# ai3DVision/CP_PFDR_graph_d1

Measured on AMD Instinct MI355X. Metric: PFDR iter/s and Medge-updates/s, 10M-vertex 6-NN graph, 1/2/4/8 MI355X, higher is better.
Workload: dtype f32; 1 GPU; PFDR_graph_quadratic_d1_l1<float>, identity A, l1 + TV, jittered 250x200x200 grid, 6-NN (V=10000000, E=60000000); global_graph=250x200x200, V_per_gpu=10000000, E_per_gpu=60000000, parallelism=single, device_inputs=True, device_bytes=3010452620, relabelled=False, split_incidence_blocks=0, tiled_blocks=39063, record_blocks=39063, slot_patterns=0, sequential_evolution=False, speculation=none, finite=True

## Files before the change

### cp_pfdr_graph_d1_amd/csrc/pfdr_quadratic.hip

```cpp
#include <cstring>
#include <map>
#include <stdexcept>


#include "pfdr_halo.hpp"
#include "pfdr_order.hpp"
#include "pfdr_quadratic_kernels.hpp"
#include "pfdr_sort.hpp"
#include "pfdr_sparse.hpp"

namespace pfdr {

template <typename real>
static void copy_in(DevBuf<real> &d, const void *src, size_t n, int mem, hipStream_t s,
                    HostPins &pins) {
    if (!src || !n) { d.release(); return; }
    d.alloc(n);
    if (mem == PFDR_MEM_DEVICE)
        PFDR_HIP(hipMemcpyAsync(d.p, src, n * sizeof(real), hipMemcpyDeviceToDevice, s));
    else
        pins.copy(d.p, src, n * sizeof(real), hipMemcpyHostToDevice);
}

template <typename real>
// ... 103 lines not shown
    long E_;
    real rho_, condMin_, difTol_, difRcd2_, cap_;
    int prox_, positivity_;
    real lo_, hi_;
    bool Ldiag_;
    bool rec_obj_, rec_dif_, track_;
    static constexpr int xcd_e_ = 64, xcd_v_ = 16;
    bool us_ = true;
    DevBuf<char> mono_ws_;
    bool la_uniform_ = false;
    real la0_ = real(0);
    bool l1_uniform_ = false;
    real l1u_ = real(0);
    const real *la_it() const { return la_uniform_ ? nullptr : La_d1_.p; }
    int evo_ = PFDR_EVOLUTION_AUTO;
    bool seqdif_ = false;
    long tstride_ = 0;
    DevBuf<real> terms_;
    DevBuf<char> dws_;
    ChainSum<real> chain_;
    TermRoute<real> route_;
    std::unique_ptr<Transport> evtr_;
    Transport &etr() { return evtr_ ? *evtr_ : *halo_->tr; }
    void seq_evolution(real *terms, const real *part, hipStream_t s);
    void sweeps(const Ctrl<real> *c);
    static constexpr int kSpecMax = 4;
    bool spec_ = false;
    int sd_ = 2;
    int it0_ = 0;
    DevBuf<R2<real>> xpx_[kSpecMax - 1];
    R2<real> *xpb(int t) { return spec_ && t % sd_ ? xpx_[t % sd_ - 1].p : xp_.p; }
    R2<real> *xr_ = nullptr, *xw_ = nullptr;
    hipStream_t evs_ = nullptr;
    hipStream_t evs() const { return evs_ ? evs_ : stream; }
    hipEvent_t evv_[kSpecMax] = {}, evd_[kSpecMax] = {};
    Ctrl<real> *snap_[2] = {};
    hipEvent_t snapev_[2] = {};
    void body_spec(int i, int n);
    static constexpr long kSeqDifMin = 1L << 17;
    std::unique_ptr<Halo> halo_;
    bool reordered_ = false;
    DevBuf<int> order_, where_, emap_;
    DevBuf<unsigned> eorig_;
    DevBuf<real> amp_orig_;
    DevBuf<int> Eu_, Ev_;
    DevBuf<real> La_d1_, La_l1_, Y_, A_, L_;
    DevBuf<R2<real>> xp_;
    DevBuf<real> diag_, Ga_, invAux_, Th_l1_, absval_, grad_, pre_, xout_;
    DevBuf<real> Z2_, wz_;
    DevBuf<real> A1_;
    DevBuf<R2<real>> gi_;
    DevBuf<real> rr_;
    int vpair_cap_ = 0;
    bool rat_on_ = false;
    real cw_ = real(0);
    DevBuf<real> R_, vpart_, opart_, Obj_, Dif_, red_, csum_;
    DevBuf<double> Rpart_;
    DevBuf<real> Rsum_, xfull_;
    DevBuf<int> lab_;
    DevBuf<real> ampg_;
    long v0_ = 0, Vglob_ = 0;
    DevBuf<long long> ccnt_;
    DevBuf<int> cnt_part_;
    DevBuf<Ctrl<real>> ctrl_;
    Incidence inc_;
    HostPins pins_;
    DevBuf<int> uptr_, blkok_;
    DevBuf<unsigned> mask_, oidx_;
    void build_split();
    bool tiled_ = false;
    DevBuf<Slots12> slots_;
    DevBuf<unsigned char> deg8_;
    DevBuf<unsigned short> luv_;
    DevBuf<int> erec_;
    DevBuf<int> ustart_, tptr_, tstart_, tlen_, tok_, trec_;
    DevBuf<Slots12> ptab_;
    DevBuf<int> prec_;
    void build_tiles();
    void build_patterns(const unsigned short *d2, long n);
    void build_tile_runs();
    Ctrl<real> *hctrl_ = nullptr;
    int nbv_, nbe_, nbn_, rows_nb_, rows_cpb_;
    int it_ = 0;
    bool stopped_ = false;
    int chunk_ = 32;
    int next_print_ = 0;
    bool graphs_ok_ = false;
    bool capturable_ = false;
    std::map<int, hipGraphExec_t> graphs_;
    void run_bodies(int n);
    hipGraphExec_t chunk_graph(int n);
  public:
    void prepare(int iters) override;
  private:
    void drop_graphs() {
        for (auto &kv : graphs_) (void)hipGraphExecDestroy(kv.second);
        graphs_.clear();
    }

    void setup_graph(const pfdr_problem *p);
    void amplitude(bool init);
    void precondition(bool init);
    void gemv_rows(int gate);
    void forward_dense(int gate);
    void gradient();
    void objective();
// ... 610 lines not shown
    k_tile_ustart<<<grid_for(Eint_ + 1), kBlock, 0, s>>>(Eint_, nb, Eu_.p, ustart_.p);
    DevBuf<int> cnt(nb), fill(nb);
    PFDR_HIP(hipMemsetAsync(cnt.p, 0, sizeof(int) * nb, s));
    PFDR_HIP(hipMemsetAsync(fill.p, 0, sizeof(int) * nb, s));
    struct Src { long n; const int *a; const unsigned long long *keys; long rs; };
    const Src src[3] = {{E_, Ev_.p, nullptr, 0},
                        {E_ - Eint_, Eu_.p + Eint_, nullptr, Eint_ - E_},
                        {R, nullptr, halo_ ? halo_->recv_keys.p : nullptr, E_}};
    for (const Src &q : src)
        if (q.n > 0) k_tile_runs_count<<<grid_for(q.n), kBlock, 0, s>>>(q.n, q.a, q.keys, V_, cnt.p);
    PFDR_HIP(hipGetLastError());
    std::vector<int> h(nb), tp((size_t)nb + 1, 0);
    PFDR_HIP(hipMemcpyAsync(h.data(), cnt.p, sizeof(int) * nb, hipMemcpyDeviceToHost, s));
    PFDR_HIP(hipStreamSynchronize(s));
    for (int b = 0; b < nb; b++) tp[b + 1] = tp[b] + h[b];
    const int nruns = tp[nb];
    tptr_.alloc((size_t)nb + 1);
    PFDR_HIP(hipMemcpyAsync(tptr_.p, tp.data(), sizeof(int) * (nb + 1), hipMemcpyHostToDevice, s));
    tstart_.alloc(nruns ? nruns : 1);
    tlen_.alloc(nruns ? nruns : 1);
    for (const Src &q : src)
        if (q.n > 0)
            k_tile_runs_fill<<<grid_for(q.n), kBlock, 0, s>>>(q.n, q.a, q.keys, V_, q.rs, tptr_.p,
                                                              fill.p, tstart_.p, tlen_.p);
    tok_.alloc(nb);
    k_tile_ok<<<grid_for(nb), kBlock, 0, s>>>(V_, nb, inc_.ptr.p, tptr_.p, kTileCap, tok_.p);
    trec_.alloc((size_t)nb * kTileRec);
    k_tile_rec<<<grid_for(nb), kBlock, 0, s>>>(nb, ustart_.p, tptr_.p, tstart_.p, tlen_.p, tok_.p,
                                               trec_.p);
    deg8_.alloc(V_);
    k_tile_deg<<<grid_for(V_), kBlock, 0, s>>>(V_, inc_.ptr.p, deg8_.p);
    PFDR_HIP(hipGetLastError());
    PFDR_HIP(hipMemcpyAsync(h.data(), tok_.p, sizeof(int) * nb, hipMemcpyDeviceToHost, s));
    PFDR_HIP(hipStreamSynchronize(s));
    long n = 0, nr = 0;
    for (int x : h) {
        n += x != 0;
        nr += x == 2;
    }
    tiled_blocks = n;
    record_blocks = nr;
    const char *e = getenv("PFDR_VPAIR");
    if (sizeof(real) == 4 && nr == nb && !(e && e[0] == '0')) {
        DevBuf<int> ent(nb);
        k_rec_entries<<<grid_for(nb), kBlock, 0, s>>>(V_, nb, inc_.ptr.p, tok_.p, ent.p);
        PFDR_HIP(hipGetLastError());
        PFDR_HIP(hipMemcpyAsync(h.data(), ent.p, sizeof(int) * nb, hipMemcpyDeviceToHost, s));
        PFDR_HIP(hipStreamSynchronize(s));
        const int cap = std::max(1, *std::max_element(h.begin(), h.end()));
        const size_t per_wg = 2 * (size_t)cap * sizeof(real) + 2048;
        if (per_wg * 7 <= 160 * 1024) vpair_cap_ = cap;
        vertex_pair = vpair_cap_;
    }
}

template <typename real>
void QuadSession<real>::build_patterns(const unsigned short *d2, long n) {
    const char *e = getenv("PFDR_TILE_PATTERNS");
    if ((e && e[0] == '0') || !record_blocks) return;
    hipStream_t s = stream;
    const int nb = grid_for(V_);
    const long nr = (long)nb * kPrec;
    std::vector<unsigned long long> hh(nr);
    std::vector<int> rec((size_t)nb * kTileRec);
    {
        DevBuf<unsigned long long> h(nr);
        k_run_hash<<<grid_for(nr), kBlock, 0, s>>>(nb, E_, tok_.p, trec_.p, d2, h.p);
        PFDR_HIP(hipGetLastError());
        PFDR_HIP(hipMemcpyAsync(hh.data(), h.p, sizeof(unsigned long long) * nr,
                                hipMemcpyDeviceToHost, s));
        PFDR_HIP(hipMemcpyAsync(rec.data(), trec_.p, sizeof(int) * rec.size(),
                                hipMemcpyDeviceToHost, s));
        PFDR_HIP(hipStreamSynchronize(s));
    }
    constexpr size_t kMaxPatterns = 65536;
    std::unordered_map<unsigned long long, int> pat;
    std::vector<long long> pA;
    std::vector<int> pLen, pOff, prec(nr, 0);
    std::vector<long long> repA(nr, -1);
    long groups = 0;
    for (long id = 0; id < nr; id++) {
        if (hh[id] == ~0ull) continue;
        auto it = pat.find(hh[id]);
        int pi;
        if (it == pat.end()) {
            const int b = (int)(id / kPrec), q = (int)(id % kPrec);
            const int *r = &rec[(size_t)b * kTileRec];
            const long long A = q == 0 ? r[0] : E_ + r[1 + 2 * q];
            const int len = q == 0 ? r[1] : r[2 + 2 * q];
            pi = (int)pA.size();
            pat.emplace(hh[id], pi);
            pA.push_back(A);
            pLen.push_back(len);
            pOff.push_back((int)groups);
            groups += ((A & 7) + len + 7) / 8;
            if (pat.size() > kMaxPatterns || groups * kSlotGroup > n / 4) return;
        } else {
            pi = it->second;
        }
        prec[id] = pOff[pi];
        repA[id] = pA[pi];
    }
    if (!groups) return;
    {
        DevBuf<long long> dr(nr);
        DevBuf<int> bad(1);
// ... 442 lines not shown
    a.late = fuse_ ? 1 : 0;
    a.E = E_;
    if (tiled_) {
        a.slots = slots_.p; a.trec = trec_.p; a.ptab = ptab_.p; a.prec = prec_.p; a.deg8 = deg8_.p; a.ustart = ustart_.p; a.tptr = tptr_.p; a.tstart = tstart_.p;
        a.tlen = tlen_.p; a.tok = tok_.p;
        a.zs = Z2_.p; a.invAux = invAux_.p; a.a0 = cw_ * la0_;
        a.gi = gi_.p;
    }
    a.l1uni = l1_uniform_ ? 1 : 0;
    a.l1u = l1u_;
    a.terms = seqdif_ ? terms_.p : nullptr;
    a.tmap = seqdif_ && reordered_ ? order_.p : nullptr;
    a.tstride = tstride_;
    a.bbeg = bbeg; a.nb = bend - bbeg; a.xcd = xcd_fit(a.nb, xcd_v_);
    a.bsplit = a.nb; a.bjump = 0;
    return a;
}

template <typename real>
void QuadSession<real>::vertex_sweep(int bbeg, int bend, const Ctrl<real> *c, const char *name,
                                     int bbeg2, int bend2) {
    if (bend <= bbeg) { bbeg = bbeg2; bend = bend2; bbeg2 = bend2 = 0; }
    if (bend <= bbeg) return;
    hipStream_t s = stream;
    VArgs<real> a = vargs(bbeg, bend, c);
    if (bend2 > bbeg2) {
        a.bsplit = bend - bbeg;
        a.bjump = bbeg2 - bend;
        a.nb += bend2 - bbeg2;
        a.xcd = xcd_fit(a.nb, xcd_v_);
    }
    ProfScope ps(prof, name, s);
    if (pad_ && bend2 <= bbeg2) {
        k_vertex_sweep_pad<real><<<xcd_grid(a.nb, a.xcd), kBlock, 0, s>>>(
            a, wzp_.p, pad_nmax_, ends_ ? pidx_.p : nullptr, ends_ ? xpe_.p : nullptr);
        return;
    }
    if (vpair_cap_ && bend2 <= bbeg2 && a.nb >= 2) {
        const int np = a.nb / 2;
        const size_t lb = 2 * (size_t)vpair_cap_ * sizeof(real);
        if (a.nb & 1) {
            VArgs<real> a1 = a;
            a1.bbeg = a.bbeg + a.nb - 1;
            a1.nb = 1;
            a1.bsplit = 1;
            a1.xcd = 0;
            if (zdirect()) k_vertex_sweep<real, 8, true><<<1, kBlock, 0, s>>>(a1);
            else k_vertex_sweep<real, 8><<<1, kBlock, 0, s>>>(a1);
        }
        a.xcd = xcd_fit(np, xcd_v_);
        const int g = xcd_grid(np, a.xcd);
        if (zdirect()) k_vertex_sweep_pair<real, true><<<g, kBlock, lb, s>>>(a, vpair_cap_);
        else k_vertex_sweep_pair<real><<<g, kBlock, lb, s>>>(a, vpair_cap_);
        return;
    }
    if (zdirect())
        k_vertex_sweep<real, 8, true><<<xcd_grid(a.nb, a.xcd), kBlock, 0, s>>>(a);
    else
        k_vertex_sweep<real, 8><<<xcd_grid(a.nb, a.xcd), kBlock, 0, s>>>(a);
}

template <typename real>
void QuadSession<real>::sweeps(const Ctrl<real> *c) {
    hipStream_t s = stream;
    if (overlap_) {
        PFDR_HIP(hipEventRecord(ev_[0], s));
        PFDR_HIP(hipStreamWaitEvent(comm_, ev_[0], 0));
        {
            ProfScope ps(prof, "halo_pull", comm_);
            halo_->pull(xr_, sizeof(R2<real>), comm_);
        }
        PFDR_HIP(hipEventRecord(ev_[1], comm_));
        edge_sweep(elo_, ehi_, c, "edge_sweep");
        PFDR_HIP(hipStreamWaitEvent(s, ev_[1], 0));
        edge_sweep(0, elo_, c, "edge_sweep_b", ehi_, E_);
        PFDR_HIP(hipEventRecord(ev_[2], s));
        PFDR_HIP(hipStreamWaitEvent(comm_, ev_[2], 0));
        {
            ProfScope ps(prof, "halo_push", comm_);
            real *src = zdirect() ? Z2_.p : wz_.p;
            halo_->push(src, src + 2 * E_, sizeof(real), comm_);
        }
        PFDR_HIP(hipEventRecord(ev_[3], comm_));
        vertex_sweep(blo_, bhi_, c, "vertex_sweep");
        PFDR_HIP(hipStreamWaitEvent(s, ev_[3], 0));
        vertex_sweep(0, blo_, c, "vertex_sweep_b", bhi_, nbv_);
    } else {
        if (halo_) {
            ProfScope ps(prof, "halo_pull", s);
            halo_->pull(xr_, sizeof(R2<real>), s);
        }
        edge_sweep(0, E_, c, "edge_sweep");
        if (halo_) {
            ProfScope ps(prof, "halo_push", s);
            real *src = zdirect() ? Z2_.p : wz_.p;
            halo_->push(src, src + 2 * E_, sizeof(real), s);
        }
        vertex_sweep(0, nbv_, c, "vertex_sweep");
    }
}

template <typename real>
void QuadSession<real>::body_spec(int i, int n) {
    hipStream_t s = stream;
    const int t = it0_ + 1 + i;
    const Ctrl<real> *c = ctrl_.p;
// ... 498 lines not shown
```

### cp_pfdr_graph_d1_amd/csrc/pfdr_quadratic_kernels.hpp

```cpp
#pragma once
#include <algorithm>
#include <cmath>
#include <cstring>
#include <memory>
#include <type_traits>

#include "pfdr_graph.hpp"
#include "pfdr_monosum.hpp"
#include "pfdr_session.hpp"

namespace pfdr {

enum AMode : int { A_IDENT = 0, A_DIAG = 1, A_DIRECT = 2, A_ATA = 3 };
enum Prox : int { PROX_NONE = 0, PROX_L1 = 1, PROX_POS = 2, PROX_BOX = 3,
                  PROX_LO = 4, PROX_HI = 5 };
enum Gate : int { GATE_NONE = 0, GATE_ACTIVE = 1, GATE_OBJ = 2,
                  GATE_ACTIVE_OR_OBJ = 3 };

template <typename real> using R2 = typename Vec<real>::v2;

template <typename T, int N>
__device__ __forceinline__ Pk<T, N> ldv(const T *p) {
    return *reinterpret_cast<const Pk<T, N> *>(p);
}
// ... 213 lines not shown
    const int ngv = nt ? rp[nt - 1] : 0;
    int lo = 0, end = nt ? rp[0] : 0, beg = 0;
    for (int b = 0; b < ngv; b += kBlock * GG) {
        Slots12 d[GG];
        Pk<real, VE> x[GG][ZV];
        long base[GG], A[GG];
        int L[GG];
#pragma unroll
        for (int u = 0; u < GG; u++) {
            const int k = min(b + u * kBlock + tid, ngv - 1);
            while (end <= k) {
                beg = end;
                end = rp[++lo];
            }
            A[u] = E + rs[lo];
            L[u] = rl[lo];
            base[u] = (A[u] / G + (k - beg)) * G;
        }
#pragma unroll
        for (int u = 0; u < GG; u++) {
            d[u] = slots[base[u] / G];
#pragma unroll
            for (int z = 0; z < ZV; z++) x[u][z] = ldv<real, VE>(wz + base[u] + z * VE);
        }
#pragma unroll
        for (int u = 0; u < GG; u++)
            if (b + u * kBlock + tid < ngv) {
#pragma unroll
                for (int q = 0; q < G; q++)
                    if (base[u] + q >= A[u] && base[u] + q < A[u] + L[u])
                        lds[slot12(d[u], q)] = x[u][q / VE].v[q % VE];
            }
    }
    __syncthreads();
    int my0 = dinc - dg;
    for (int q = 0; q < w; q++) my0 += wt[q];
    const int my1 = my0 + dg;
    real s = real(0);
    int j = my0;
    for (; j + 4 <= my1; j += 4) {
        const real a0 = lds[j], a1 = lds[j + 1], a2 = lds[j + 2], a3 = lds[j + 3];
        s += ZD ? wv * a0 : a0;
        s += ZD ? wv * a1 : a1;
        s += ZD ? wv * a2 : a2;
        s += ZD ? wv * a3 : a3;
    }
    for (; j < my1; j++) s += ZD ? wv * lds[j] : lds[j];
    return s;
}

constexpr int kRecRuns = 14, kTileRec = 32;
constexpr int kPrec = 16;

template <typename real, bool ZD = false>
__device__ __forceinline__ real tile_sum_rec(int V, long E, int blk, int v,
                                             const unsigned char *__restrict__ deg8,
                                             const Slots12 *__restrict__ slots,
                                             const int *__restrict__ trec,
                                             const real *__restrict__ wz, real *lds, int *wt,
                                             real wv = real(1),
                                             const Slots12 *__restrict__ ptab = nullptr,
                                             const int *__restrict__ prec = nullptr,
                                             bool pre = false, int pre_rv = 0, int pre_pr = 0,
                                             int pre_dg = 0) {
    constexpr int VE = Vec<real>::kPer16B, G = kSlotGroup, ZV = G / VE;
    const int tid = threadIdx.x, lane = tid & (kWave - 1), w = tid / kWave;
    const int dg = pre ? pre_dg : v < V ? deg8[v] : 0;
    const int rv = pre ? pre_rv : lane < kTileRec ? trec[(long)blk * kTileRec + lane] : 0;
    const int pr = pre ? pre_pr : prec && lane < kPrec ? prec[(long)blk * kPrec + lane] : 0;
    int dinc = dg;
#pragma unroll
    for (int o = 1; o < kWave; o <<= 1) {
        const int y = __shfl_up(dinc, o, kWave);
        if (lane >= o) dinc += y;
    }
    if (lane == kWave - 1) wt[w] = dinc;
    const int us = __builtin_amdgcn_readlane(rv, 0), nu = __builtin_amdgcn_readlane(rv, 1);
    const int nt = __builtin_amdgcn_readlane(rv, 2);
    const int st = __shfl(rv, min(3 + 2 * lane, kWave - 1), kWave);
    const int ln = __shfl(rv, min(4 + 2 * lane, kWave - 1), kWave);
    int P = 0;
    if (lane < nt && ln > 0) {
        const long A = E + st;
        P = (int)((A + ln - 1) / G - A / G + 1);
    }
#pragma unroll
    for (int o = 1; o < kWave; o <<= 1) {
        const int y = __shfl_up(P, o, kWave);
        if (lane >= o) P += y;
    }
    const int ngv = __builtin_amdgcn_readlane(P, kWave - 1);
    const long fu = us / G;
    const int ngu = nu > 0 ? (int)((us + nu - 1) / G - fu + 1) : 0;
    const int tot = ngu + ngv;
    for (int b = 0; b < tot; b += 2 * kBlock) {
        Slots12 d[2];
        Pk<real, VE> x[2][ZV];
        long gb[2], lo[2], hi[2];
        int pg[2];
#pragma unroll
        for (int u = 0; u < 2; u++) {
            const int k = min(b + u * kBlock + tid, tot - 1);
            const int kv = k - ngu;
            int r = 0;
            for (int q = 0; q < nt; q++) r += __builtin_amdgcn_readlane(P, q) <= kv;
            r = min(r, kWave - 1);
            const int sr = __shfl(st, r, kWave), lr = __shfl(ln, r, kWave);
            const int pb = __shfl(P, max(r - 1, 0), kWave);
            const int pv = __shfl(pr, min(r + 1, kWave - 1), kWave);
            if (k < ngu) {
                gb[u] = fu + k;
                lo[u] = us;
                hi[u] = (long)us + nu;
                pg[u] = __builtin_amdgcn_readlane(pr, 0) + k;
            } else {
                const long A = E + sr;
                const int gi = kv - (r > 0 ? pb : 0);
                gb[u] = A / G + gi;
                lo[u] = A;
                hi[u] = A + lr;
                pg[u] = pv + gi;
            }
        }
#pragma unroll
        for (int u = 0; u < 2; u++) {
            d[u] = prec ? ptab[pg[u]] : slots[gb[u]];
#pragma unroll
            for (int z = 0; z < ZV; z++) x[u][z] = ldv<real, VE>(wz + gb[u] * G + z * VE);
        }
#pragma unroll
        for (int u = 0; u < 2; u++)
            if (b + u * kBlock + tid < tot) {
#pragma unroll
                for (int q = 0; q < G; q++) {
                    const long p = gb[u] * G + q;
                    if (p >= lo[u] && p < hi[u]) lds[slot12(d[u], q)] = x[u][q / VE].v[q % VE];
                }
            }
    }
    __syncthreads();
    int my0 = dinc - dg;
    for (int q = 0; q < w; q++) my0 += wt[q];
    const int my1 = my0 + dg;
    real s = real(0);
    int j = my0;
    for (; j + 4 <= my1; j += 4) {
        const real a0 = lds[j], a1 = lds[j + 1], a2 = lds[j + 2], a3 = lds[j + 3];
        s += ZD ? wv * a0 : a0;
        s += ZD ? wv * a1 : a1;
        s += ZD ? wv * a2 : a2;
        s += ZD ? wv * a3 : a3;
    }
    for (; j < my1; j++) s += ZD ? wv * lds[j] : lds[j];
    return s;
}

template <typename real, bool ZD = false>
__device__ __forceinline__ void tile_sum_rec2(int V, long E, int b0, int v0, int v1,
                                              const unsigned char *__restrict__ deg8,
                                              const Slots12 *__restrict__ slots,
                                              const int *__restrict__ trec,
                                              const real *__restrict__ wz, real *lds, int cap,
                                              int *wt, real wv0, real wv1,
                                              const Slots12 *__restrict__ ptab,
                                              const int *__restrict__ prec, real &x0, real &x1) {
    static_assert(kTileRec == 32 && kWave == 64 && kPrec == 16, "two records per wave register");
    constexpr int VE = Vec<real>::kPer16B, G = kSlotGroup, ZV = G / VE, NW = kBlock / kWave;
    const int tid = threadIdx.x, lane = tid & (kWave - 1), w = tid / kWave;
    const int dg0 = v0 < V ? deg8[v0] : 0, dg1 = v1 < V ? deg8[v1] : 0;
    const int rv = trec[(long)b0 * kTileRec + lane];
    const int pr = prec ? prec[(long)b0 * kPrec + (lane & 31)] : 0;
    int i0 = dg0, i1 = dg1;
#pragma unroll
    for (int o = 1; o < kWave; o <<= 1) {
        const int y0 = __shfl_up(i0, o, kWave), y1 = __shfl_up(i1, o, kWave);
        if (lane >= o) {
            i0 += y0;
            i1 += y1;
        }
    }
    if (lane == kWave - 1) {
        wt[w] = i0;
        wt[NW + w] = i1;
    }
    const int us0 = __builtin_amdgcn_readlane(rv, 0), nu0 = __builtin_amdgcn_readlane(rv, 1);
    const int nt0 = __builtin_amdgcn_readlane(rv, 2);
    const int us1 = __builtin_amdgcn_readlane(rv, 32), nu1 = __builtin_amdgcn_readlane(rv, 33);
    const int nt1 = __builtin_amdgcn_readlane(rv, 34);
    const int hf = lane >> 5, rl = lane & 31;
    const int st = __shfl(rv, 32 * hf + min(3 + 2 * rl, 31), kWave);
    const int ln = __shfl(rv, 32 * hf + min(4 + 2 * rl, 31), kWave);
    int P = 0;
    if (rl < (hf ? nt1 : nt0) && ln > 0) {
        const long A = E + st;
        P = (int)((A + ln - 1) / G - A / G + 1);
    }
#pragma unroll
    for (int o = 1; o < 32; o <<= 1) {
        const int y = __shfl_up(P, o, kWave);
        if (rl >= o) P += y;
    }
    const int ngv0 = __builtin_amdgcn_readlane(P, 31), ngv1 = __builtin_amdgcn_readlane(P, 63);
    const long fu0 = us0 / G, fu1 = us1 / G;
    const int ngu0 = nu0 > 0 ? (int)((us0 + nu0 - 1) / G - fu0 + 1) : 0;
    const int ngu1 = nu1 > 0 ? (int)((us1 + nu1 - 1) / G - fu1 + 1) : 0;
    const int tot0 = ngu0 + ngv0, tot = tot0 + ngu1 + ngv1;
    const int pu0 = __builtin_amdgcn_readlane(pr, 0), pu1 = __builtin_amdgcn_readlane(pr, 16);
// ... 1557 lines not shown
                pd.wzp[pd.sl[2 * e]] = ou;
                pd.wzp[pd.sl[2 * e + 1]] = ov;
            } else {
                wz[e] = ou;
                wz[E + e] = ov;
            }
        }
    }
}

template <typename real>
struct VArgs {
    int V;
    int nb, xcd;
    int bbeg;
    int bsplit, bjump;
    const int *ptr;
    const unsigned *idx;
    const int *uptr;
    const unsigned *mask, *oidx;
    const int *blkok;
    const real *wz;
    R2<real> *xp;
    R2<real> *xpo;
    const real *Y, *A, *Ga, *Th_l1;
    int prox, positivity;
    real lo, hi;
    int fwd;
    int track;
    real *part;
    const Ctrl<real> *ctrl;
    int late;
    long E;
    const Slots12 *slots;
    const int *trec;
    const Slots12 *ptab;
    const int *prec;
    const unsigned char *deg8;
    const int *ustart, *tptr, *tstart, *tlen, *tok;
    const real *zs;
    const real *invAux;
    real a0;
    const R2<real> *gi;
    int l1uni;
    real l1u;
    real *terms;
    const int *tmap;
    long tstride;
};

template <typename real> struct VSweep;
template <> struct VSweep<float> { static constexpr int waves = 8; };
template <> struct VSweep<double> { static constexpr int waves = 4; };

template <typename real>
struct VOps {
    R2<real> q{};
    real th = real(0), yv = real(0), gv = real(0), av = real(0), ia = real(0);
};
template <typename real>
__device__ __forceinline__ VOps<real> vertex_ops(const VArgs<real> &a, int v,
                                                 const R2<real> *gpre = nullptr) {
    VOps<real> o;
    if (v < a.V) {
        if (a.track || !a.fwd) o.q = a.xp[v];
        real g = real(0);
        if (a.gi) {
            const R2<real> p = gpre ? *gpre : a.gi[v];
            g = p.x;
            o.ia = p.y;
        } else if (a.fwd || a.l1uni) {
            g = a.Ga[v];
        }
        if (a.prox == PROX_L1) o.th = a.l1uni ? g * a.l1u : a.Th_l1[v];
        if (a.fwd) { o.yv = a.Y[v]; o.gv = g; }
        if (a.fwd == 2) o.av = a.A[v];
    }
    return o;
}

template <typename real>
__device__ __forceinline__ R2<real> vertex_finish(const VArgs<real> &a, int v, real x,
                                                  const VOps<real> &o, real &num, real &den) {
    num = real(0);
    den = real(0);
    R2<real> q = o.q;
    const real th = o.th, yv = o.yv, gv = o.gv, av = o.av;
    if (v < a.V) {
        switch (a.prox) {
            case PROX_L1: {
                if (x > th) x -= th;
                else if (!a.positivity && (x < -th)) x += th;
                else x = real(0);
            } break;
            case PROX_POS:
                if (x < real(0)) x = real(0);
                break;
            case PROX_BOX:
                if (x < a.lo) x = a.lo;
                else if (x > a.hi) x = a.hi;
                break;
            case PROX_LO:
                if (x < a.lo) x = a.lo;
                break;
            case PROX_HI:
                if (x > a.hi) x = a.hi;
// ... 15 lines not shown
        if (a.fwd) {
            real p = (a.fwd == 2) ? av * x : x;
            p -= yv;
            q.y = real(2) * x - gv * p;
        }
        (a.xpo ? a.xpo : a.xp)[v] = q;
    }
    return q;
}

template <typename real, int GB, bool ZD = false>
__device__ __forceinline__ void vertex_block(const VArgs<real> &a, int blk, real *lds,
                                             real (*red)[kBlock / kWave], int *scan,
                                             int halt = 0) {
    const int v0 = blk * kBlock;
    const int v = v0 + threadIdx.x;
    const VOps<real> o = vertex_ops(a, v);
    const real wv = ZD && v < a.V ? a.a0 * (a.gi ? o.ia : a.invAux[v]) : real(1);
    real x;
    const bool pre = a.slots && a.trec;
    int pre_rv = 0, pre_pr = 0, pre_dg = 0;
    if (pre) {
        const int lane = threadIdx.x & (kWave - 1);
        pre_rv = lane < kTileRec ? a.trec[(long)blk * kTileRec + lane] : 0;
        pre_pr = a.prec && lane < kPrec ? a.prec[(long)blk * kPrec + lane] : 0;
        pre_dg = v < a.V ? a.deg8[v] : 0;
    }
    const int tk = a.slots ? a.tok[blk] : 0;
    if (tk == 2)
        x = tile_sum_rec<real, ZD>(a.V, a.E, blk, v, a.deg8, a.slots, a.trec, ZD ? a.zs : a.wz,
                                   lds, scan + 3 * kTileRuns, wv, a.ptab, a.prec, pre, pre_rv,
                                   pre_pr, pre_dg);
    else if (tk)
        x = tile_sum<real, GB, ZD>(a.V, a.E, blk, v, a.deg8, a.slots, a.ustart, a.tptr, a.tstart,
                                   a.tlen, ZD ? a.zs : a.wz, lds, scan, wv);
    else if (!ZD && a.blkok && a.blkok[blk])
        x = split_sum<real, GB>(a.V, v0, v, a.ptr, a.uptr, a.mask, a.oidx, a.wz, lds, scan);
    else
        x = gather_sum<real, GatherCap<real>::v, GB, ZD>(a.V, v0, a.ptr, a.idx,
                                                         ZD ? a.zs : a.wz, lds, wv);
    if (halt) return;
    real num, den;
    vertex_finish(a, v, x, o, num, den);
    if (a.track) {
        num = block_sum(num, red[0]);
        den = block_sum(den, red[1]);
        if (threadIdx.x == 0) {
            a.part[2 * blk] = num;
            a.part[2 * blk + 1] = den;
        }
    }
}

template <typename real, int GB, bool ZD = false>
__global__ __launch_bounds__(256, VSweep<real>::waves) void k_vertex_sweep(VArgs<real> a) {
    int halt = 0;
    if (a.ctrl) {
        if (!a.late) {
            if (a.ctrl->halt) return;
        } else {
            halt = a.ctrl->halt;
        }
    }
    __shared__ real lds[GatherCap<real>::v];
    __shared__ real red[2][kBlock / kWave];
    __shared__ int scan[3 * kTileRuns + kBlock / kWave];
    int lb = xcd_block(blockIdx.x, a.nb, a.xcd);
    if (lb >= a.nb) return;
    lb = a.nb - 1 - lb;
    if (lb >= a.bsplit) lb += a.bjump;
    vertex_block<real, GB, ZD>(a, a.bbeg + lb, lds, red, scan, halt);
}

template <typename real, bool ZD = false>
__global__ __launch_bounds__(256, 7) void k_vertex_sweep_pair(VArgs<real> a, int cap) {
    int halt = 0;
    if (a.ctrl) {
        if (!a.late) {
            if (a.ctrl->halt) return;
        } else {
            halt = a.ctrl->halt;
        }
    }
    extern __shared__ __attribute__((aligned(16))) unsigned char vpair_lds[];
    real *lds = reinterpret_cast<real *>(vpair_lds);
    __shared__ real red[2][kBlock / kWave];
    __shared__ int scan[3 * kTileRuns + 2 * (kBlock / kWave)];
    const int np = a.nb / 2;
    int lp = xcd_block(blockIdx.x, np, a.xcd);
    if (lp >= np) return;
    lp = np - 1 - lp;
    const int b0 = a.bbeg + 2 * lp;
    const int v0 = b0 * kBlock + threadIdx.x, v1 = v0 + kBlock;
    const VOps<real> o0 = vertex_ops(a, v0);
    const real wv0 = ZD && v0 < a.V ? a.a0 * (a.gi ? o0.ia : a.invAux[v0]) : real(1);
    real x0, x1;
    R2<real> g1{};
    if (a.gi && v1 < a.V) g1 = a.gi[v1];
    const real wv1 = ZD && v1 < a.V ? a.a0 * (a.gi ? g1.y : a.invAux[v1]) : real(1);
    tile_sum_rec2<real, ZD>(a.V, a.E, b0, v0, v1, a.deg8, a.slots, a.trec, ZD ? a.zs : a.wz, lds,
                            cap, scan + 3 * kTileRuns, wv0, wv1, a.ptab, a.prec, x0, x1);
    if (halt) return;
    const VOps<real> o1 = vertex_ops(a, v1, a.gi ? &g1 : nullptr);
    real n0, d0, n1, d1;
    vertex_finish(a, v0, x0, o0, n0, d0);
    vertex_finish(a, v1, x1, o1, n1, d1);
    if (a.track) {
        n0 = block_sum(n0, red[0]);
        d0 = block_sum(d0, red[1]);
        n1 = block_sum(n1, red[0]);
        d1 = block_sum(d1, red[1]);
        if (threadIdx.x == 0) {
            a.part[2 * b0] = n0;
            a.part[2 * b0 + 1] = d0;
            a.part[2 * b0 + 2] = n1;
            a.part[2 * b0 + 3] = d1;
        }
    }
}
// ... 445 lines not shown
```

### cp_pfdr_graph_d1_amd/csrc/pfdr_runtime.cpp

```cpp
#include <chrono>
#include <hip/hip_runtime.h>

#include <cstdarg>
#include <cstring>
#include <map>
#include <mutex>
#include <string>

#include "pfdr_session.hpp"

namespace pfdr {

static thread_local std::string g_last_error;

static void set_error(const char *fmt, ...) {
    char buf[1024];
    va_list ap;
    va_start(ap, fmt);
    vsnprintf(buf, sizeof buf, fmt, ap);
    va_end(ap);
    g_last_error = buf;
}

static double now_ms() {
// ... 434 lines not shown
            size_t b = n.find(',', a);
            if (b == std::string::npos) b = n.size();
            if (b > a) o.push_back(n.substr(a, b - a));
            a = b + 1;
        }
    }
    return PFDR_OK;
}

extern "C" int pfdr_session_set_profiling(pfdr_session *s, int on) {
    if (!s) return report_error("pfdr_session_set_profiling", "null session");
    PFDR_GUARD("pfdr_session_set_profiling", {
        s->impl->prof.on = (on != 0);
        s->impl->prof.period = on > 1 ? on : 1;
        if (on) s->impl->prof.reserve(1024);
    });
    return PFDR_OK;
}

extern "C" int pfdr_session_kernel_stats(pfdr_session *s, const char *kernel,
                                         int *launches, double *mean_ms) {
    if (!s || !kernel || !launches || !mean_ms)
        return report_error("pfdr_session_kernel_stats", "null argument");
    PFDR_GUARD("pfdr_session_kernel_stats", {
        StreamScope sc(s->impl->stream, s->impl->device);
        PFDR_HIP(hipStreamSynchronize(s->impl->stream));
        s->impl->prof.resolve();
        s->impl->prof.stats(kernel, launches, mean_ms);
    });
    return PFDR_OK;
}

extern "C" int pfdr_session_sync(pfdr_session *s) {
    if (!s) return report_error("pfdr_session_sync", "null session");
    PFDR_GUARD("pfdr_session_sync", {
        PFDR_HIP(hipStreamSynchronize(s->impl->stream));
    });
    return PFDR_OK;
}

extern "C" int64_t pfdr_session_device_bytes(pfdr_session *s) {
    return s ? s->impl->device_bytes : -1;
}

extern "C" int pfdr_session_query(pfdr_session *s, const char *what, int64_t *value) {
    if (!s || !what || !value) return report_error("pfdr_session_query", "null argument");
    if (!strcmp(what, "reordered")) *value = s->impl->reordered;
    else if (!strcmp(what, "split_blocks")) *value = s->impl->split_blocks;
    else if (!strcmp(what, "tiled_blocks")) *value = s->impl->tiled_blocks;
    else if (!strcmp(what, "record_blocks")) *value = s->impl->record_blocks;
    else if (!strcmp(what, "slot_patterns")) *value = s->impl->slot_patterns;
    else if (!strcmp(what, "edge_ratio")) *value = s->impl->edge_ratio;
    else if (!strcmp(what, "vertex_pair")) *value = s->impl->vertex_pair;
    else if (!strcmp(what, "ustaged")) *value = s->impl->ustaged;
    else if (!strcmp(what, "symv")) *value = s->impl->symv;
    else if (!strcmp(what, "tiny")) *value = s->impl->tiny;
    else if (!strcmp(what, "fused")) *value = s->impl->fused;
    else if (!strcmp(what, "padded")) *value = s->impl->padded;
    else if (!strcmp(what, "seqdif")) *value = s->impl->seqdif;
    else if (!strcmp(what, "la_uniform")) *value = s->impl->la_uniform;
    else if (!strcmp(what, "ghosts")) *value = s->impl->ghosts;
    else if (!strcmp(what, "graphs")) *value = s->impl->graphs;
    else if (!strcmp(what, "speculative")) *value = s->impl->speculative;
    else if (!strcmp(what, "dense_exact")) *value = s->impl->dense_exact;
    else if (!strcmp(what, "sparse_exact")) *value = s->impl->sparse_exact;
    else if (!strcmp(what, "sparse_nnz")) *value = s->impl->sparse_nnz;
    else if (!strcmp(what, "sparse_seg_col")) *value = s->impl->sparse_seg_col;
    else if (!strcmp(what, "sparse_seg_row")) *value = s->impl->sparse_seg_row;
    else if (!strcmp(what, "sparse_csr_us")) *value = s->impl->sparse_csr_us;
    else if (!strcmp(what, "interior_edges")) *value = s->impl->interior_edges;
    else if (!strcmp(what, "device_bytes")) *value = s->impl->device_bytes;
    else return report_error("pfdr_session_query", (std::string("unknown key ") + what).c_str());
    return PFDR_OK;
}

extern "C" void pfdr_session_destroy(pfdr_session *s) {
    if (!s) return;
    try {
        StreamScope sc(s->impl->stream, s->impl->device);
        (void)hipStreamSynchronize(s->impl->stream);
        delete s->impl;
    } catch (...) {
    }
    delete s;
}
```

### cp_pfdr_graph_d1_amd/csrc/pfdr_session.hpp

```cpp
#pragma once
#include <map>
#include <stdexcept>
#include <string>
#include <vector>

#include "pfdr_dev.hpp"

namespace pfdr {

class Profiler {
  public:
    bool on = false;
    int period = 1;
    std::vector<std::string> only;
    ~Profiler();
    bool begin(const char *name, hipStream_t s);
    void end(hipStream_t s);
    void resolve();
    void reserve(int n);
    bool stats(const char *name, int *launches, double *mean_ms) const;

  private:
    struct Pending { int id; hipEvent_t a, b; };
    std::vector<Pending> pend_;
    std::vector<hipEvent_t> pool_;
    std::map<std::string, int> ids_;
    std::vector<double> total_ms_;
    std::vector<int> count_, seen_;
    int open_id_ = -1;
    hipEvent_t open_ev_ = nullptr;
    hipEvent_t take();
};

struct ProfScope {
    Profiler &p;
    hipStream_t s;
    bool on;
    ProfScope(Profiler &pr, const char *name, hipStream_t st)
        : p(pr), s(st), on(pr.on && pr.begin(name, st)) {}
    ~ProfScope() { if (on) p.end(s); }
};

class SessionBase {
  public:
    virtual ~SessionBase() = default;
    virtual int run(int iters) = 0;
    virtual void result(void *X_host, int *it, void *Obj_host,
                        void *Dif_host) = 0;
    virtual void *device_x() = 0;
    virtual void prepare(int iters) { (void)iters; }
    int64_t device_bytes = 0;
    int64_t reordered = 0;
    int64_t split_blocks = 0;
    int64_t tiled_blocks = 0;
    int64_t record_blocks = 0;
    int64_t slot_patterns = 0;
    int64_t edge_ratio = 0;
    int64_t vertex_pair = 0;
    int64_t ustaged = 0;
    int64_t symv = 0;
    int64_t tiny = 0;
    int64_t fused = 0;
    int64_t padded = 0;
    int64_t seqdif = 0;
    int64_t la_uniform = 0;
    int64_t dense_exact = 0;
    int64_t sparse_exact = 0;
    int64_t sparse_nnz = 0;
    int64_t sparse_seg_col = 0, sparse_seg_row = 0;
    int64_t sparse_csr_us = 0;
    virtual bool sparse_csr(int64_t *, int32_t *, void *) { return false; }
    int64_t ghosts = 0;
    int64_t graphs = 0;
    int64_t speculative = 0;
    int64_t interior_edges = -1;
    hipStream_t stream = nullptr;
    Profiler prof;
    int device = 0;
};

inline int spec_mode(const pfdr_problem *p) {
    const char *e = getenv("PFDR_SPEC");
    int m = p->spec;
    if (e && *e) {
        const std::string v(e);
        if (v == "auto") m = PFDR_SPEC_AUTO;
        else if (v == "serial") m = PFDR_SPEC_SERIAL;
        else if (v == "off") m = PFDR_SPEC_OFF;
        else throw std::runtime_error("PFDR_SPEC must be auto, serial or off");
    }
    if (m < PFDR_SPEC_AUTO || m > PFDR_SPEC_OFF)
        throw std::runtime_error("spec must be PFDR_SPEC_AUTO, _SERIAL or _OFF");
    return m;
}

struct CallTrace {
    const char *fn;
    bool on;
    double t0, t_setup = 0, t_run = 0;
    explicit CallTrace(const char *name);
    void setup_done();
    void run_done();
    void finish(long V, long E, long N, int K, int it);
};

std::vector<int> multidev_devices(const pfdr_problem *p);
void multidev_solve(const pfdr_problem *p, const std::vector<int> &devs, int *it, void *Obj,
                    void *Dif);

}

// ... 4 lines not shown
```

Measured before the change: 146,300 Medge-updates/s.

## Process two vertex blocks per workgroup, prefetching second block's records during first

```diff
diff --git a/cp_pfdr_graph_d1_amd/csrc/pfdr_quadratic.hip b/cp_pfdr_graph_d1_amd/csrc/pfdr_quadratic.hip
--- a/cp_pfdr_graph_d1_amd/csrc/pfdr_quadratic.hip
+++ b/cp_pfdr_graph_d1_amd/csrc/pfdr_quadratic.hip
@@ -179,6 +179,7 @@
     DevBuf<R2<real>> gi_;
     DevBuf<real> rr_;
     int vpair_cap_ = 0;
+    bool vseq2_ = false;
     bool rat_on_ = false;
     real cw_ = real(0);
     DevBuf<real> R_, vpart_, opart_, Obj_, Dif_, red_, csum_;
@@ -895,6 +896,9 @@
         if (per_wg * 7 <= 160 * 1024) vpair_cap_ = cap;
         vertex_pair = vpair_cap_;
     }
+    const char *e2 = getenv("PFDR_VSEQ2");
+    vseq2_ = !halo_ && nb >= 2 && nr == nb && !vpair_cap_ && !(e2 && e2[0] == '0');
+    vertex_seq2 = vseq2_ ? 1 : 0;
 }
 
 template <typename real>
@@ -1443,6 +1447,29 @@
         const int g = xcd_grid(np, a.xcd);
         if (zdirect()) k_vertex_sweep_pair<real, true><<<g, kBlock, lb, s>>>(a, vpair_cap_);
         else k_vertex_sweep_pair<real><<<g, kBlock, lb, s>>>(a, vpair_cap_);
+        return;
+    }
+    if (vseq2_ && bend2 <= bbeg2 && a.nb >= 2) {
+        const int np = a.nb / 2;
+        if (a.nb & 1) {
+            VArgs<real> a1 = a;
+            a1.bbeg = a.bbeg + a.nb - 1;
+            a1.nb = 1;
+            a1.bsplit = 1;
+            a1.xcd = 0;
+            if (zdirect()) k_vertex_sweep<real, 8, true><<<1, kBlock, 0, s>>>(a1);
+            else k_vertex_sweep<real, 8><<<1, kBlock, 0, s>>>(a1);
+        }
+        a.xcd = xcd_fit(np, xcd_v_);
+        const int g = xcd_grid(np, a.xcd);
+        const bool lean = !a.track && a.fwd == 1 && !a.terms;
+        if (zdirect()) {
+            if (lean) k_vertex_sweep<real, 8, true, 2><<<g, kBlock, 0, s>>>(a);
+            else k_vertex_sweep<real, 8, true, 1><<<g, kBlock, 0, s>>>(a);
+        } else {
+            if (lean) k_vertex_sweep<real, 8, false, 2><<<g, kBlock, 0, s>>>(a);
+            else k_vertex_sweep<real, 8, false, 1><<<g, kBlock, 0, s>>>(a);
+        }
         return;
     }
     if (zdirect())
diff --git a/cp_pfdr_graph_d1_amd/csrc/pfdr_quadratic_kernels.hpp b/cp_pfdr_graph_d1_amd/csrc/pfdr_quadratic_kernels.hpp
--- a/cp_pfdr_graph_d1_amd/csrc/pfdr_quadratic_kernels.hpp
+++ b/cp_pfdr_graph_d1_amd/csrc/pfdr_quadratic_kernels.hpp
@@ -289,6 +289,135 @@
 constexpr int kRecRuns = 14, kTileRec = 32;
 constexpr int kPrec = 16;
 
+struct RecRuns {
+    int st, ln;
+    int P;
+    int pr;
+};
+struct RecBlk {
+    int us, nu, nt;
+    int ngu, ngv, tot;
+    int pu;
+    long fu;
+};
+
+template <bool HALF>
+__device__ __forceinline__ void rec_decode(long E, int rv, int pr, RecRuns &t, RecBlk *hb) {
+    static_assert(kTileRec == 32 && kWave == 64 && kPrec == 16, "two records per wave register");
+    constexpr int G = kSlotGroup, W = HALF ? kTileRec : kWave, NB = HALF ? 2 : 1;
+    const int lane = threadIdx.x & (kWave - 1);
+    const int hf = HALF ? lane >> 5 : 0, rl = HALF ? lane & 31 : lane;
+#pragma unroll
+    for (int h = 0; h < NB; h++) {
+        hb[h].us = __builtin_amdgcn_readlane(rv, kTileRec * h);
+        hb[h].nu = __builtin_amdgcn_readlane(rv, kTileRec * h + 1);
+        hb[h].nt = __builtin_amdgcn_readlane(rv, kTileRec * h + 2);
+        hb[h].pu = __builtin_amdgcn_readlane(pr, kPrec * h);
+    }
+    t.pr = pr;
+    t.st = __shfl(rv, W * hf + min(3 + 2 * rl, W - 1), kWave);
+    t.ln = __shfl(rv, W * hf + min(4 + 2 * rl, W - 1), kWave);
+    int P = 0;
+    if (rl < (hf ? hb[NB - 1].nt : hb[0].nt) && t.ln > 0) {
+        const long A = E + t.st;
+        P = (int)((A + t.ln - 1) / G - A / G + 1);
+    }
+#pragma unroll
+    for (int o = 1; o < W; o <<= 1) {
+        const int y = __shfl_up(P, o, kWave);
+        if (rl >= o) P += y;
+    }
+    t.P = P;
+#pragma unroll
+    for (int h = 0; h < NB; h++) {
+        hb[h].ngv = __builtin_amdgcn_readlane(P, W * h + W - 1);
+        hb[h].fu = hb[h].us / G;
+        hb[h].ngu =
+            hb[h].nu > 0 ? (int)((hb[h].us + hb[h].nu - 1) / G - hb[h].fu + 1) : 0;
+        hb[h].tot = hb[h].ngu + hb[h].ngv;
+    }
+}
+
+template <typename real>
+struct RecChunk {
+    Slots12 d[2];
+    Pk<real, Vec<real>::kPer16B> x[2][kSlotGroup / Vec<real>::kPer16B];
+    int mt[2];
+};
+
+template <typename real, int H>
+__device__ __forceinline__ void rec_load(const RecRuns &t, const RecBlk &hb, long E, int b,
+                                         const Slots12 *__restrict__ slots,
+                                         const Slots12 *__restrict__ ptab, bool pat,
+                                         const real *__restrict__ wz, RecChunk<real> &c) {
+    constexpr int VE = Vec<real>::kPer16B, G = kSlotGroup, ZV = G / VE;
+    constexpr int base = kTileRec * H, pbase = kPrec * H;
+    long gb[2];
+    int pg[2];
+#pragma unroll
+    for (int u = 0; u < 2; u++) {
+        const int k = min(b + u * kBlock + (int)threadIdx.x, hb.tot - 1);
+        const int kv = k - hb.ngu;
+        int r = 0;
+        for (int q = 0; q < hb.nt; q++) r += __builtin_amdgcn_readlane(t.P, base + q) <= kv;
+        r = min(r, kTileRec - 1);
+        const int sr = __shfl(t.st, base + r, kWave), lr = __shfl(t.ln, base + r, kWave);
+        const int pb = __shfl(t.P, base + max(r - 1, 0), kWave);
+        const int pv = __shfl(t.pr, pbase + min(r + 1, kPrec - 1), kWave);
+        long lo, hi;
+        if (k < hb.ngu) {
+            gb[u] = hb.fu + k;
+            lo = hb.us;
+            hi = (long)hb.us + hb.nu;
+            pg[u] = hb.pu + k;
+        } else {
+            const long A = E + sr;
+            const int gi = kv - (r > 0 ? pb : 0);
+            gb[u] = A / G + gi;
+            lo = A;
+            hi = A + lr;
+            pg[u] = pv + gi;
+        }
+        const int l = (int)max(lo - gb[u] * G, -1L), h = (int)min(hi - gb[u] * G, (long)G + 1);
+        c.mt[u] = (l + 1) | (h + 1) << 4;
+    }
+#pragma unroll
+    for (int u = 0; u < 2; u++) {
+        c.d[u] = pat ? ptab[pg[u]] : slots[gb[u]];
+#pragma unroll
+        for (int z = 0; z < ZV; z++) c.x[u][z] = ldv<real, VE>(wz + gb[u] * G + z * VE);
+    }
+}
+
+template <typename real>
+__device__ __forceinline__ void rec_scatter(const RecChunk<real> &c, int b, int tot, real *lds) {
+    constexpr int VE = Vec<real>::kPer16B, G = kSlotGroup;
+#pragma unroll
+    for (int u = 0; u < 2; u++)
+        if (b + u * kBlock + (int)threadIdx.x < tot) {
+            const int lo = (c.mt[u] & 15) - 1, hi = ((c.mt[u] >> 4) & 15) - 1;
+#pragma unroll
+            for (int q = 0; q < G; q++)
+                if (q >= lo && q < hi) lds[slot12(c.d[u], q)] = c.x[u][q / VE].v[q % VE];
+        }
+}
+
+template <typename real, bool ZD>
+__device__ __forceinline__ real list_walk(const real *lds, int my0, int dg, real wv) {
+    const int my1 = my0 + dg;
+    real s = real(0);
+    int j = my0;
+    for (; j + 4 <= my1; j += 4) {
+        const real a0 = lds[j], a1 = lds[j + 1], a2 = lds[j + 2], a3 = lds[j + 3];
+        s += ZD ? wv * a0 : a0;
+        s += ZD ? wv * a1 : a1;
+        s += ZD ? wv * a2 : a2;
+        s += ZD ? wv * a3 : a3;
+    }
+    for (; j < my1; j++) s += ZD ? wv * lds[j] : lds[j];
+    return s;
+}
+
 template <typename real, bool ZD = false>
 __device__ __forceinline__ real tile_sum_rec(int V, long E, int blk, int v,
                                              const unsigned char *__restrict__ deg8,
@@ -300,7 +429,6 @@
                                              const int *__restrict__ prec = nullptr,
                                              bool pre = false, int pre_rv = 0, int pre_pr = 0,
                                              int pre_dg = 0) {
-    constexpr int VE = Vec<real>::kPer16B, G = kSlotGroup, ZV = G / VE;
     const int tid = threadIdx.x, lane = tid & (kWave - 1), w = tid / kWave;
     const int dg = pre ? pre_dg : v < V ? deg8[v] : 0;
     const int rv = pre ? pre_rv : lane < kTileRec ? trec[(long)blk * kTileRec + lane] : 0;
@@ -312,84 +440,18 @@
         if (lane >= o) dinc += y;
     }
     if (lane == kWave - 1) wt[w] = dinc;
-    const int us = __builtin_amdgcn_readlane(rv, 0), nu = __builtin_amdgcn_readlane(rv, 1);
-    const int nt = __builtin_amdgcn_readlane(rv, 2);
-    const int st = __shfl(rv, min(3 + 2 * lane, kWave - 1), kWave);
-    const int ln = __shfl(rv, min(4 + 2 * lane, kWave - 1), kWave);
-    int P = 0;
-    if (lane < nt && ln > 0) {
-        const long A = E + st;
-        P = (int)((A + ln - 1) / G - A / G + 1);
-    }
-#pragma unroll
-    for (int o = 1; o < kWave; o <<= 1) {
-        const int y = __shfl_up(P, o, kWave);
-        if (lane >= o) P += y;
-    }
-    const int ngv = __builtin_amdgcn_readlane(P, kWave - 1);
-    const long fu = us / G;
-    const int ngu = nu > 0 ? (int)((us + nu - 1) / G - fu + 1) : 0;
-    const int tot = ngu + ngv;
-    for (int b = 0; b < tot; b += 2 * kBlock) {
-        Slots12 d[2];
-        Pk<real, VE> x[2][ZV];
-        long gb[2], lo[2], hi[2];
-        int pg[2];
-#pragma unroll
-        for (int u = 0; u < 2; u++) {
-            const int k = min(b + u * kBlock + tid, tot - 1);
-            const int kv = k - ngu;
-            int r = 0;
-            for (int q = 0; q < nt; q++) r += __builtin_amdgcn_readlane(P, q) <= kv;
-            r = min(r, kWave - 1);
-            const int sr = __shfl(st, r, kWave), lr = __shfl(ln, r, kWave);
-            const int pb = __shfl(P, max(r - 1, 0), kWave);
-            const int pv = __shfl(pr, min(r + 1, kWave - 1), kWave);
-            if (k < ngu) {
-                gb[u] = fu + k;
-                lo[u] = us;
-                hi[u] = (long)us + nu;
-                pg[u] = __builtin_amdgcn_readlane(pr, 0) + k;
-            } else {
-                const long A = E + sr;
-                const int gi = kv - (r > 0 ? pb : 0);
-                gb[u] = A / G + gi;
-                lo[u] = A;
-                hi[u] = A + lr;
-                pg[u] = pv + gi;
-            }
-        }
-#pragma unroll
-        for (int u = 0; u < 2; u++) {
-            d[u] = prec ? ptab[pg[u]] : slots[gb[u]];
-#pragma unroll
-            for (int z = 0; z < ZV; z++) x[u][z] = ldv<real, VE>(wz + gb[u] * G + z * VE);
-        }
-#pragma unroll
-        for (int u = 0; u < 2; u++)
-            if (b + u * kBlock + tid < tot) {
-#pragma unroll
-                for (int q = 0; q < G; q++) {
-                    const long p = gb[u] * G + q;
-                    if (p >= lo[u] && p < hi[u]) lds[slot12(d[u], q)] = x[u][q / VE].v[q % VE];
-                }
-            }
+    RecRuns t;
+    RecBlk hb;
+    rec_decode<false>(E, rv, pr, t, &hb);
+    for (int b = 0; b < hb.tot; b += 2 * kBlock) {
+        RecChunk<real> c;
+        rec_load<real, 0>(t, hb, E, b, slots, ptab, prec != nullptr, wz, c);
+        rec_scatter(c, b, hb.tot, lds);
     }
     __syncthreads();
     int my0 = dinc - dg;
     for (int q = 0; q < w; q++) my0 += wt[q];
-    const int my1 = my0 + dg;
-    real s = real(0);
-    int j = my0;
-    for (; j + 4 <= my1; j += 4) {
-        const real a0 = lds[j], a1 = lds[j + 1], a2 = lds[j + 2], a3 = lds[j + 3];
-        s += ZD ? wv * a0 : a0;
-        s += ZD ? wv * a1 : a1;
-        s += ZD ? wv * a2 : a2;
-        s += ZD ? wv * a3 : a3;
-    }
-    for (; j < my1; j++) s += ZD ? wv * lds[j] : lds[j];
-    return s;
+    return list_walk<real, ZD>(lds, my0, dg, wv);
 }
 
 template <typename real, bool ZD = false>
@@ -2053,6 +2115,10 @@
 template <typename real> struct VSweep;
 template <> struct VSweep<float> { static constexpr int waves = 8; };
 template <> struct VSweep<double> { static constexpr int waves = 4; };
+template <typename real, bool LEAN> struct VSeq2;
+template <> struct VSeq2<float, false> { static constexpr int waves = 7; };
+template <> struct VSeq2<float, true> { static constexpr int waves = 8; };
+template <bool LEAN> struct VSeq2<double, LEAN> { static constexpr int waves = 4; };
 
 template <typename real>
 struct VOps {
@@ -2174,8 +2240,89 @@
     }
 }
 
-template <typename real, int GB, bool ZD = false>
-__global__ __launch_bounds__(256, VSweep<real>::waves) void k_vertex_sweep(VArgs<real> a) {
+template <typename real>
+__device__ __forceinline__ VArgs<real> lean_args(VArgs<real> a) {
+    a.track = 0;
+    a.fwd = 1;
+    a.terms = nullptr;
+    return a;
+}
+
+template <typename real, bool ZD, bool LEAN>
+__device__ __forceinline__ void vertex_seq2(const VArgs<real> &a_in, int b0, real *lds,
+                                            real (*red)[kBlock / kWave], int *wt0, int *wt1,
+                                            int halt) {
+    const VArgs<real> a = LEAN ? lean_args(a_in) : a_in;
+    const int tid = threadIdx.x, lane = tid & (kWave - 1), w = tid / kWave;
+    const int v0 = b0 * kBlock + tid, v1 = v0 + kBlock;
+    const int rv = a.trec[(long)b0 * kTileRec + lane];
+    const int pr = a.prec ? a.prec[(long)b0 * kPrec + (lane & 31)] : 0;
+    const int dg0 = v0 < a.V ? a.deg8[v0] : 0, dg1 = v1 < a.V ? a.deg8[v1] : 0;
+    const VOps<real> o0 = vertex_ops(a, v0), o1 = vertex_ops(a, v1);
+    const real wv0 = ZD && v0 < a.V ? a.a0 * (a.gi ? o0.ia : a.invAux[v0]) : real(1);
+    const real wv1 = ZD && v1 < a.V ? a.a0 * (a.gi ? o1.ia : a.invAux[v1]) : real(1);
+    int i0 = dg0, i1 = dg1;
+#pragma unroll
+    for (int o = 1; o < kWave; o <<= 1) {
+        const int y0 = __shfl_up(i0, o, kWave), y1 = __shfl_up(i1, o, kWave);
+        if (lane >= o) {
+            i0 += y0;
+            i1 += y1;
+        }
+    }
+    if (lane == kWave - 1) {
+        wt0[w] = i0;
+        wt1[w] = i1;
+    }
+    RecRuns t;
+    RecBlk hb[2];
+    rec_decode<true>(a.E, rv, pr, t, hb);
+    const real *wz = ZD ? a.zs : a.wz;
+    const bool pat = a.prec != nullptr;
+    for (int b = 0; b < hb[0].tot; b += 2 * kBlock) {
+        RecChunk<real> c;
+        rec_load<real, 0>(t, hb[0], a.E, b, a.slots, a.ptab, pat, wz, c);
+        rec_scatter(c, b, hb[0].tot, lds);
+    }
+    __syncthreads();
+    RecChunk<real> c1;
+    if (hb[1].tot > 0) rec_load<real, 1>(t, hb[1], a.E, 0, a.slots, a.ptab, pat, wz, c1);
+    int my0 = i0 - dg0, my1 = i1 - dg1;
+    for (int q = 0; q < w; q++) {
+        my0 += wt0[q];
+        my1 += wt1[q];
+    }
+    const real x0 = list_walk<real, ZD>(lds, my0, dg0, wv0);
+    __syncthreads();
+    if (hb[1].tot > 0) rec_scatter(c1, 0, hb[1].tot, lds);
+    for (int b = 2 * kBlock; b < hb[1].tot; b += 2 * kBlock) {
+        RecChunk<real> c;
+        rec_load<real, 1>(t, hb[1], a.E, b, a.slots, a.ptab, pat, wz, c);
+        rec_scatter(c, b, hb[1].tot, lds);
+    }
+    __syncthreads();
+    const real x1 = list_walk<real, ZD>(lds, my1, dg1, wv1);
+    if (halt) return;
+    real n0, d0, n1, d1;
+    vertex_finish(a, v0, x0, o0, n0, d0);
+    vertex_finish(a, v1, x1, o1, n1, d1);
+    if (a.track) {
+        n0 = block_sum(n0, red[0]);
+        d0 = block_sum(d0, red[1]);
+        n1 = block_sum(n1, red[0]);
+        d1 = block_sum(d1, red[1]);
+        if (tid == 0) {
+            a.part[2 * b0] = n0;
+            a.part[2 * b0 + 1] = d0;
+            a.part[2 * b0 + 2] = n1;
+            a.part[2 * b0 + 3] = d1;
+        }
+    }
+}
+
+template <typename real, int GB, bool ZD = false, int SEQ2 = 0>
+__global__ __launch_bounds__(256, (SEQ2 ? VSeq2<real, SEQ2 == 2>::waves : VSweep<real>::waves))
+void k_vertex_sweep(VArgs<real> a) {
     int halt = 0;
     if (a.ctrl) {
         if (!a.late) {
@@ -2187,6 +2334,15 @@
     __shared__ real lds[GatherCap<real>::v];
     __shared__ real red[2][kBlock / kWave];
     __shared__ int scan[3 * kTileRuns + kBlock / kWave];
+    if constexpr (SEQ2) {
+        const int np = a.nb / 2;
+        int lp = xcd_block(blockIdx.x, np, a.xcd);
+        if (lp >= np) return;
+        lp = np - 1 - lp;
+        vertex_seq2<real, ZD, SEQ2 == 2>(a, a.bbeg + 2 * lp, lds, red, scan + 3 * kTileRuns, scan,
+                                         halt);
+        return;
+    }
     int lb = xcd_block(blockIdx.x, a.nb, a.xcd);
     if (lb >= a.nb) return;
     lb = a.nb - 1 - lb;
diff --git a/cp_pfdr_graph_d1_amd/csrc/pfdr_runtime.cpp b/cp_pfdr_graph_d1_amd/csrc/pfdr_runtime.cpp
--- a/cp_pfdr_graph_d1_amd/csrc/pfdr_runtime.cpp
+++ b/cp_pfdr_graph_d1_amd/csrc/pfdr_runtime.cpp
@@ -510,6 +510,7 @@
     else if (!strcmp(what, "slot_patterns")) *value = s->impl->slot_patterns;
     else if (!strcmp(what, "edge_ratio")) *value = s->impl->edge_ratio;
     else if (!strcmp(what, "vertex_pair")) *value = s->impl->vertex_pair;
+    else if (!strcmp(what, "vertex_seq2")) *value = s->impl->vertex_seq2;
     else if (!strcmp(what, "ustaged")) *value = s->impl->ustaged;
     else if (!strcmp(what, "symv")) *value = s->impl->symv;
     else if (!strcmp(what, "tiny")) *value = s->impl->tiny;
diff --git a/cp_pfdr_graph_d1_amd/csrc/pfdr_session.hpp b/cp_pfdr_graph_d1_amd/csrc/pfdr_session.hpp
--- a/cp_pfdr_graph_d1_amd/csrc/pfdr_session.hpp
+++ b/cp_pfdr_graph_d1_amd/csrc/pfdr_session.hpp
@@ -57,6 +57,7 @@
     int64_t slot_patterns = 0;
     int64_t edge_ratio = 0;
     int64_t vertex_pair = 0;
+    int64_t vertex_seq2 = 0;
     int64_t ustaged = 0;
     int64_t symv = 0;
     int64_t tiny = 0;
```

Result: slower. 143,700 Medge-updates/s (-1.8%).
